# mit-han-lab/litepose

Hardware: AMD Instinct MI355X
Metric: images/sec end-to-end (backbone+deconv+AE-group), LitePose-XS@256 b64 (higher is better)
Workload: dtype f32

## Files before the change

### litepose_amd/csrc/engine.cpp

```cpp
#include <hip/hip_runtime.h>

#include <cmath>
#include <cstdio>
#include <cstdint>
#include <cstring>
#include <map>
#include <string>
#include <vector>

#include "../../include/litepose_amd.h"
#include "kernels.h"
#include "plan.h"

using namespace lp_plan;

namespace {

thread_local std::string g_err;
int fail(int code, const std::string& msg) {
    g_err = msg;
    return code;
}
#define HIP_OK(expr)                                                                   \
    do {                                                                               \
        hipError_t e_ = (expr);                                                        \
        if (e_ != hipSuccess)                                                          \
            return fail(LP_ERR_HIP, std::string(#expr) + ": " + hipGetErrorString(e_)); \
    } while (0)

static_assert(ACT_NONE == lp::ACT_NONE && ACT_RELU == lp::ACT_RELU && ACT_RELU6 == lp::ACT_RELU6, "plan.h restates lp::Act");

const char* storage_name(const Net* n) { return n->storage == LP_STORAGE_F16 ? "f16" : "bf16"; }

}

struct lp_net : lp_plan::Net {
    bool finalized = false;
    float* d_weights = nullptr;
    std::vector<char*> last_buf;
    int lastN = 0, lastH = 0, lastW = 0;
    bool profiling = false;
    std::vector<hipEvent_t> events;
    struct ProfEntry { std::string name, kernel; int64_t bytes, flops; int ev0, ev1; int64_t flops_valu; lp::LaunchNote launch; };
    std::vector<ProfEntry> prof_entries;
    int prof_ev = 0;
    static constexpr int MAX_SIDE = 8;
    hipStream_t side[MAX_SIDE] = {};
    hipEvent_t ev_fork = nullptr, ev_join[MAX_SIDE] = {};
    int nstreams = 0;
    int opt_mb16 = 1;
    int opt_mb16_run = 1;
    int opt_mb16_min = 48;
    int opt_mbt = 1, opt_mbt_s2 = 1;
    int opt_mbconv2 = 1;
    int opt_mbtb = 1, opt_mbtb_s2 = 1;
    int opt_pw3d = 1;
    int opt_mbtd = 1;
    int opt_mbtq = 1;
    int opt_headb = 1;
    int opt_headfuse = 1;
    int opt_dwt = 2;
    int opt_stem = 1;
    int opt_diag_dwpw = 0;
    struct OptEntryT { const char* key; int lo, hi; int lp_net::*field; };
    static const std::vector<OptEntryT>& options();
    std::vector<char> last_stored;
    struct CalibLayer { std::string bn; int C, div; size_t off; };
    struct Calib {
        lp_net* raw = nullptr;
        std::vector<CalibLayer> layers;
        std::map<std::string, int> index;
        std::vector<float> h_bn;
        float* d_bn = nullptr;
        double momentum = 0.1;
        int64_t steps = 0;
        bool uploaded = false;
    };
    Calib* calib = nullptr;
};

namespace {

size_t buf_elems(const lp_net* n, int b, int N, int H, int W, size_t esz) {
    const int d = n->bufs.div[b];
    const size_t f = (size_t)N * n->bufs.ch[b] * (H / d) * (W / d), q = 256 / esz;
    return (f + q - 1) / q * q;
}
size_t buf_floats(const lp_net* n, int b, int N, int H, int W) { return buf_elems(n, b, N, H, W, sizeof(float)); }

size_t buf_bytes(const lp_net* n, int b, int N, int H, int W) {
    const size_t esz = n->storage != LP_STORAGE_F32 ? sizeof(uint16_t) : sizeof(float);
    return buf_elems(n, b, N, H, W, esz) * esz;
}

int size_multiple(const lp_net* n) {
    int m = 16;
    for (int d : n->bufs.div) m = std::max(m, d);
    return m;
}

int check_size(const lp_net* n, int H, int W) {
    const int m = size_multiple(n);
    if (H < m || W < m || (H % m) || (W % m))
        return fail(LP_ERR_INVALID_ARG, "H and W must be positive multiples of " + std::to_string(m) +
                                            " (the deepest plane of this net is 1/" + std::to_string(m) + " of the input)");
    return LP_OK;
}

}

extern "C" {

const char* lp_last_error(void) { return g_err.c_str(); }
void lp_set_error_(const char* msg) { g_err = msg ? msg : ""; }
const char* lp_version(void) { return "litepose_amd 0.1 (gfx950, fp32 planar)"; }

int lp_net_create(lp_net** out, const lp_arch* a) {
    if (!out || !a) return fail(LP_ERR_INVALID_ARG, "null argument");
    lp_net* n = new lp_net();
    if (const int rc = init_arch(*n, *a)) {
        delete n;
        return fail(rc, lp_plan::last_error());
    }
    *out = n;
    return LP_OK;
}

static void calib_release(lp_net* n) {
    if (!n->calib) return;
    if (n->calib->d_bn) (void)hipFree(n->calib->d_bn);
    lp_net_destroy(n->calib->raw);
    delete n->calib;
    n->calib = nullptr;
}

void lp_net_destroy(lp_net* n) {
// ... 183 lines not shown
    const float* Wt;
    bool f32, f16;
    float* f(int b) const { return reinterpret_cast<float*>(buf[b]); }
    const OpBase& op(size_t i) const { return f32 ? static_cast<const OpBase&>(n->ops[i]) : n->bops[i]; }
    Cost cost(size_t i, CostPart part = COST_OP) const {
        return f32 ? op_cost(n->ops[i], 4, false, NB, H, W, part) : op_cost(n->bops[i], 2, n->bops[i].out_f32, NB, H, W);
    }
    int mark(const std::string& name, const Cost& k) const { return prof_mark(n, s, name, k); }
};
struct Planes { int ih, iw, oh, ow; };
Planes planes(const Part& c, const OpBase& o) { return {c.H / o.in_div, c.W / o.in_div, c.H / o.out_div, c.W / o.out_div}; }

struct Rule {
    int (*launch)(const Part&, size_t i);
    std::string (*name)(const OpBase& first, const OpBase& second, const OpBase& last);
    int64_t (*bytes)(const Part&, size_t i);
};

std::string block_name(const OpBase& o, const OpBase& d, const OpBase& last) {
    const std::string nm = o.name + "+" + d.name.substr(d.name.rfind('.', d.name.find('+')) + 1);
    if (&last == &d) return nm;
    const std::string pfx = o.name.substr(0, o.name.rfind('.'));
    const std::string lpf = last.name.substr(0, last.name.rfind('.', last.name.find('+')));
    return pfx + "-" + lpf.substr(lpf.rfind('.') + 1) + nm.substr(pfx.size());
}
std::string blockb_name(const OpBase& o, const OpBase&, const OpBase&) { return o.name + "+dw+point_conv"; }
std::string stem_name(const OpBase&, const OpBase&, const OpBase&) { return "stem.conv3x3s2+dw3+pw"; }
std::string dwpw3_name(const OpBase& dw, const OpBase&, const OpBase&) { return dw.name + "+pw"; }
std::string headb_name(const OpBase&, const OpBase& second, const OpBase& pw) {
    return "final." + pw.name.substr(6, pw.name.find('.', 6) - 6) + (&second == &pw ? ".dw5+pw" : ".dw5+dw5+pw");
}
std::string head_name(const OpBase& dw, const OpBase& second, const OpBase& pw) {
    if (&second != &pw && dw.name.substr(0, dw.name.find('.')) != "final_refined") return pw.name;
    return headb_name(dw, second, pw);
}
std::string half_name(const OpBase& d, CostPart part) {
    if (part == COST_DW_HALF) return d.name.substr(0, d.name.find('+'));
    return d.name.substr(0, d.name.rfind('.', d.name.find('+'))) + ".point_conv";
}


bool is_block(const std::vector<Op>& ops, size_t i) {
    return ops[i].type == OP_PW && ops[i].fuse_next && i + 1 < ops.size() && ops[i + 1].type == OP_DWPW;
}

int rule_mb16(const Part& c, size_t i) {
    const lp_net* n = c.n;
    if (!is_block(n->ops, i)) return 0;
    const Op &o = n->ops[i], &d = n->ops[i + 1];
    const Planes pl = planes(c, o);
    if (!(n->opt_mb16 && c.NB >= n->opt_mb16_min && o.ws_off && d.ws_off && d.wrow_off &&
          lp::mb16_supported(o.Ca, o.Cout, d.Cout, pl.ih, pl.iw, d.K, d.S, d.res >= 0)))
        return 0;
    const float* Wt = c.Wt;
    lp::Mb16Run r;
    memset(&r, 0, sizeof(r));
    for (size_t k = i; k + 1 < n->ops.size() && r.nblocks < lp::MB16_MAX_RUN; k += 2) {
        const Op &e = n->ops[k], &p = n->ops[k + 1];
        if (e.type != OP_PW || !e.fuse_next || p.type != OP_DWPW || !e.ws_off || !p.ws_off || !p.wrow_off) break;
        if (k > i) {
            if (d.res < 0 || p.res != e.inA || e.inA != n->ops[k - 1].out || e.Ca != o.Ca ||
                e.Cout != o.Cout || p.Cout != d.Cout || p.K != d.K || p.S != d.S ||
                e.in_div != o.in_div || p.out_div != d.out_div || !n->opt_mb16_run)
                break;
        } else if (d.res >= 0 && d.res != o.inA) break;
        const int b = r.nblocks++;
        r.w1s[b] = Wt + e.ws_off; r.b1f[b] = Wt + e.b_off; r.wrow[b] = Wt + p.wrow_off;
        r.w2s[b] = Wt + p.ws_off; r.b2f[b] = Wt + p.b2_off; r.out[b] = c.f(p.out);
        if (d.res < 0) break;
    }
    if (r.nblocks < 1 || !lp::launch_mb16(c.f(o.inA), r, d.res >= 0, c.NB, o.Ca, o.Cout, d.Cout, pl.ih, pl.iw, d.K, d.S, c.s))
        return 0;
    return 2 * r.nblocks;
}

int rule_mbt(const Part& c, size_t i) {
    const lp_net* n = c.n;
    if (!is_block(n->ops, i)) return 0;
    const Op &o = n->ops[i], &d = n->ops[i + 1];
    const Planes pl = planes(c, o);
    const float *Wt = c.Wt, *res = d.res >= 0 ? c.f(d.res) : nullptr;
    return ((o.ws_off && d.ws_off && d.wrow_off &&
             lp::launch_mbt(c.f(o.inA), Wt + o.ws_off, Wt + o.b_off, Wt + d.wrow_off, Wt + d.ws_off, Wt + d.b2_off, res,
                            c.f(d.out), c.NB, o.Ca, o.Cout, d.Cout, pl.ih, pl.iw, d.K, d.S, c.s, n->opt_mbt, n->opt_mbt_s2)) ||
            lp::launch_mbconv(c.f(o.inA), Wt + o.w_off, Wt + o.b_off, Wt + d.w_off, Wt + d.b_off, Wt + d.w2_off,
                              Wt + d.b2_off, res, c.f(d.out), c.NB, o.Ca, o.Cout, d.Cout, pl.ih, pl.iw, d.K, d.S, c.s,
                              d.wpair_off ? Wt + d.wpair_off : nullptr, o.ws_off ? Wt + o.ws_off : nullptr,
                              d.wrow_off ? Wt + d.wrow_off : nullptr, n->opt_mbconv2)) ? 2 : 0;
}

int rule_stem3(const Part& c, size_t i) {
    const lp_net* n = c.n;
    const Op& o = n->ops[i];
    if (!(n->opt_stem && o.type == OP_STEM && i + 2 < n->ops.size() && n->ops[i + 1].type == OP_DW &&
          n->ops[i + 2].type == OP_PW && o.st_w0))
        return 0;
    const Op &dw = n->ops[i + 1], &pw = n->ops[i + 2];
    const float* Wt = c.Wt;
    return lp::launch_stem3(c.x, Wt + o.st_w0, Wt + o.b_off, Wt + o.st_w1, Wt + dw.b_off, Wt + o.st_w2, Wt + o.st_b2,
                            c.f(pw.out), c.NB, c.H, c.W, pw.Cout, c.flip_from, c.x_batch, c.s) ? 3 : 0;
}

int rule_dwpw3(const Part& c, size_t i) {
    const lp_net* n = c.n;
    const Op& o = n->ops[i];
    if (!(o.type == OP_DW && o.K == 3 && o.S == 1 && o.act == lp::ACT_RELU6 && i + 1 < n->ops.size())) return 0;
    const Op& pw = n->ops[i + 1];
    if (!(pw.type == OP_PW && pw.inA == o.out && pw.inB < 0 && pw.res < 0 && pw.act == lp::ACT_NONE && pw.has_bias)) return 0;
    const Planes pl = planes(c, o);
    const float* Wt = c.Wt;
    return lp::launch_dwpw(c.f(o.inA), Wt + o.w_off, Wt + o.b_off, Wt + pw.w_off, Wt + pw.b_off, nullptr, c.f(pw.out), c.NB,
                           o.Ca, pl.ih, pl.iw, o.K, o.S, pw.Cout, c.s, n->opt_diag_dwpw) ? 2 : 0;
}

int rule_head(const Part& c, size_t i) {
    const lp_net* n = c.n;
    const std::vector<Op>& ops = n->ops;
    const Op& o = ops[i];
    if (!(n->opt_headfuse && o.type == OP_DW && o.S == 1 && o.act == lp::ACT_RELU && i + 1 < ops.size())) return 0;
    const Op& a = ops[i + 1];
    const Op *d2 = nullptr, *pw = nullptr;
    if (o.K == 5 && a.type == OP_PW && a.inA == o.out && a.inB < 0 && a.res < 0 && a.act == lp::ACT_NONE &&
        (a.out == n->out0_buf || a.out == n->out1_buf))
        pw = &a;
    else if (i + 2 < ops.size() && a.type == OP_DW && ops[i + 2].type == OP_PW && ops[i + 2].inA == o.out &&
             ops[i + 2].inB == a.out && a.S == 1 && o.K == a.K && a.act == lp::ACT_RELU)
        d2 = &a, pw = &ops[i + 2];
    else
        return 0;
    const Planes pl = planes(c, o);
    const float* Wt = c.Wt;
    if (!lp::launch_headfuse(c.f(o.inA), o.Ca, d2 ? c.f(d2->inA) : nullptr, d2 ? d2->Ca : 0,
                             o.wpair_off ? Wt + o.wpair_off : nullptr, d2 && d2->wpair_off ? Wt + d2->wpair_off : nullptr,
                             Wt + pw->w_off, c.f(pw->out), c.NB, pl.oh, pl.ow, o.K, pw->Cout, c.s))
        return 0;
    return d2 ? 3 : 2;
}

const Rule F32_RULES[] = {{rule_mb16, block_name, nullptr}, {rule_mbt, block_name, nullptr}, {rule_stem3, stem_name, nullptr},
                          {rule_dwpw3, dwpw3_name, nullptr}, {rule_head, head_name, nullptr}};

int launch_op_f32(const Part& c, size_t i) {
    const lp_net* n = c.n;
    const Op& o = n->ops[i];
    const Planes pl = planes(c, o);
    const int ih = pl.ih, iw = pl.iw, oh = pl.oh, ow = pl.ow, NB = c.NB;
    const float* Wt = c.Wt;
    hipStream_t s = c.s;
    switch (o.type) {
        case OP_STEM:
            lp::launch_stem(c.x, Wt + o.w_off, Wt + o.b_off, c.f(o.out), NB, c.H, c.W, c.flip_from, c.x_batch, s);
            break;
        case OP_DW:
            lp::launch_dw(c.f(o.inA), Wt + o.w_off, Wt + o.wdup_off, Wt + o.b_off, c.f(o.out), NB, o.Ca, ih, iw, o.K, o.S,
                          o.act, s);
            break;
        case OP_PW:
            lp::launch_pw(c.f(o.inA), o.Ca, o.inB >= 0 ? c.f(o.inB) : nullptr, o.Cb, Wt + o.w_off,
                          o.has_bias ? Wt + o.b_off : nullptr, o.res >= 0 ? c.f(o.res) : nullptr, c.f(o.out), NB, oh * ow,
                          o.Cout, o.act, s, o.ws_off ? Wt + o.ws_off : nullptr, n->opt_pw3d);
            break;
        case OP_DECONV: {
            float* inB = o.inB >= 0 ? c.f(o.inB) : nullptr;
            if (o.w3_off && deconv4_enabled() && o.w4_off &&
                lp::launch_deconv4x3(c.f(o.inA), o.Ca, inB, o.Cb, Wt + o.w4_off, Wt + o.b3_off, c.f(o.out), NB, ih, iw,
                                     o.Cout, s)) {
            } else if (o.w3_off && deconv4_enabled())
// ... 360 lines not shown
    if (steps_out) *steps_out = steps;
    if (steps > 0) return lp_net_finalize(n, 1);
    return LP_OK;
}

static const OpBase* find_tap(const lp_net* n, const char* name) {
    const OpBase* hit = nullptr;
    auto match = [&](const OpBase& o) { if (!hit && (o.tap == name || o.name == name)) hit = &o; };
    for (const Op& o : n->ops) match(o);
    for (const BOp& o : n->bops) if (!o.out_f32) match(o);
    return hit;
}

int64_t lp_net_tap(const lp_net* n, const char* name, float* d_dst, void* stream) {
    if (!n || !name || n->last_buf.empty()) return fail(LP_ERR_INVALID_ARG, "no forward has run");
    const OpBase* o = find_tap(n, name);
    if (!o) return fail(LP_ERR_UNKNOWN_KEY, std::string("unknown tap ") + name);
    const int d = n->bufs.div[o->out];
    const int hw = (n->lastH / d) * (n->lastW / d);
    const int64_t cnt = (int64_t)n->lastN * n->bufs.ch[o->out] * hw;
    if (n->storage != LP_STORAGE_F32) {
        if ((size_t)o->out >= n->last_stored.size() || !n->last_stored[o->out])
            return fail(LP_ERR_UNSUPPORTED, std::string("tap ") + name + ": the last forward did not store this "
                        "tensor (it lives inside a fused block launch; option \"mbtb\" = 0 runs one launch per op)");
        if (d_dst)
            lp::launch_octet_to_planar(n->last_buf[o->out], d_dst, n->lastN, n->bufs.ch[o->out], hw,
                                       (hipStream_t)stream, n->storage == LP_STORAGE_F16);
    } else if (d_dst) {
        hipError_t e = hipMemcpyAsync(d_dst, n->last_buf[o->out], (size_t)cnt * sizeof(float),
                                      hipMemcpyDeviceToDevice, (hipStream_t)stream);
        if (e != hipSuccess) return fail(LP_ERR_HIP, hipGetErrorString(e));
    }
    return cnt;
}

int64_t lp_net_tap_offset(const lp_net* n, const char* name, int NB, int H, int W, int64_t* count) {
    if (!n || !name || !n->finalized) return fail(LP_ERR_INVALID_ARG, "net not finalized");
    if (n->storage != LP_STORAGE_F32) return fail(LP_ERR_UNSUPPORTED, "fp32 storage only");
    if (NB < 1) return fail(LP_ERR_INVALID_ARG, "NB must be positive");
    if (const int rc = check_size(n, H, W)) return rc;
    const OpBase* o = find_tap(n, name);
    if (!o) return fail(LP_ERR_UNKNOWN_KEY, std::string("unknown tap ") + name);
    if (o->out == n->out0_buf || o->out == n->out1_buf) return fail(LP_ERR_UNSUPPORTED, "caller-owned output");
    size_t off = 0;
    for (int b = 0; b < o->out; ++b) off += buf_floats(n, b, NB, H, W);
    const int d = n->bufs.div[o->out];
    if (count) *count = (int64_t)NB * n->bufs.ch[o->out] * (H / d) * (W / d);
    return (int64_t)(off * sizeof(float));
}

int lp_net_set_storage(lp_net* n, int storage) {
    if (!n || (storage != LP_STORAGE_F32 && storage != LP_STORAGE_BF16 && storage != LP_STORAGE_F16))
        return fail(LP_ERR_INVALID_ARG, "storage must be LP_STORAGE_F32, LP_STORAGE_BF16 or LP_STORAGE_F16");
    if (n->calib) return fail(LP_ERR_INVALID_ARG, "a calibration is open on this handle: lp_calib_end() first");
    if (n->arch.family == 1 && storage != LP_STORAGE_F32)
        return fail(LP_ERR_UNSUPPORTED, "lp_net_set_storage: the pose_resnet family (lp_arch.family = 1) runs in fp32 storage "
                                        "only: its dense k x k convolutions have no 16-bit kernels yet");
    if (storage != n->storage) {
        n->storage = storage;
        n->finalized = false;
        n->last_buf.clear();
    }
    return LP_OK;
}

int lp_net_get_storage(const lp_net* n) { return n ? n->storage : LP_ERR_INVALID_ARG; }

int lp_round16(const float* src, float* dst, int64_t count, int storage) {
    if ((!src || !dst) && count > 0) return fail(LP_ERR_INVALID_ARG, "null argument");
    if (storage != LP_STORAGE_BF16 && storage != LP_STORAGE_F16)
        return fail(LP_ERR_INVALID_ARG, "storage must be LP_STORAGE_BF16 or LP_STORAGE_F16");
    for (int64_t i = 0; i < count; ++i) dst[i] = round16(storage, src[i]);
    return LP_OK;
}

typedef lp_net::OptEntryT OptEntry;
const std::vector<OptEntry>& lp_net::options() {
    static const std::vector<OptEntry> t = {
        {"mb16", 0, 1, &lp_net::opt_mb16},
        {"mb16_run", 0, 1, &lp_net::opt_mb16_run},
        {"mb16_min", 0, 65536, &lp_net::opt_mb16_min},
        {"mbt", 0, 3, &lp_net::opt_mbt},
        {"mbt_s2", 0, 1, &lp_net::opt_mbt_s2},
        {"mbconv2", 0, 1, &lp_net::opt_mbconv2},
        {"mbtb", 0, 1, &lp_net::opt_mbtb},
        {"mbtb_s2", 0, 1, &lp_net::opt_mbtb_s2},
        {"mbtq", 0, 2, &lp_net::opt_mbtq},
        {"mbtd", 0, 1, &lp_net::opt_mbtd},
        {"pw3d", 0, 2, &lp_net::opt_pw3d},
        {"headb", 0, 1, &lp_net::opt_headb},
        {"headfuse", 0, 1, &lp_net::opt_headfuse},
        {"dwt", 0, 2, &lp_net::opt_dwt},
        {"stem", 0, 1, &lp_net::opt_stem},
        {"diag_dwpw", 0, 2, &lp_net::opt_diag_dwpw},
    };
    return t;
}

int lp_net_set_option(lp_net* n, const char* key, int value) {
    if (!n || !key) return fail(LP_ERR_INVALID_ARG, "null argument");
    for (const OptEntry& e : lp_net::options())
        if (!strcmp(key, e.key)) {
            if (value < e.lo || value > e.hi) return fail(LP_ERR_INVALID_ARG, std::string("option ") + key + ": value out of range");
#ifndef LP_DIAG_BUILD
            if (e.field == &lp_net::opt_diag_dwpw && value != 0)
                return fail(LP_ERR_UNSUPPORTED, "option diag_dwpw: the self-checking dwpw_kernel exists only in the diagnostics "
                                                "flavour of the library (python -m litepose_amd.build --flavour diag, "
                                                "LP_NATIVE_FLAVOUR=diag)");
#endif
            n->*(e.field) = value;
            return LP_OK;
        }
    return fail(LP_ERR_UNKNOWN_KEY, std::string("unknown option ") + key);
}

int lp_net_get_option(const lp_net* n, const char* key) {
    if (!n || !key) return fail(LP_ERR_INVALID_ARG, "null argument");
    for (const OptEntry& e : lp_net::options())
        if (!strcmp(key, e.key)) return n->*(e.field);
    return fail(LP_ERR_UNKNOWN_KEY, std::string("unknown option ") + key);
}

int lp_diag_read(uint32_t* words, int cap_words, int clear) {
    const int n = lp::dwpw_diag_read(words, cap_words, clear != 0);
    if (n == -2) return fail(LP_ERR_UNSUPPORTED, "lp_diag_read: no diagnostic kernel in this library (build --flavour diag)");
    if (n < 0) return fail(LP_ERR_HIP, "lp_diag_read: copy from the device log failed");
    return n;
}

int lp_phase_trace_read(uint64_t* words, int nwg) {
    static_assert(sizeof(unsigned long long) == sizeof(uint64_t), "");
    const int n = lp::phase_trace_read(reinterpret_cast<unsigned long long*>(words), nwg);
    if (n == -2) return fail(LP_ERR_UNSUPPORTED, "lp_phase_trace_read: no phase trace in this library (build --flavour trace)");
    if (n < 0) return fail(LP_ERR_HIP, "lp_phase_trace_read: bad count / copy from the device table failed");
    return n;
}

int lp_wg_trace_read(uint64_t* words, int nwg, int select_cexp) {
    if (nwg < 0 || nwg > 16384) return fail(LP_ERR_INVALID_ARG, "lp_wg_trace_read: 0..16384 workgroups");
    const int n = lp::wg_trace_read(reinterpret_cast<unsigned long long*>(words), nwg, select_cexp);
    if (n == -2) return fail(LP_ERR_UNSUPPORTED, "lp_wg_trace_read: no trace in this library (build --flavour trace)");
    if (n < 0) return fail(LP_ERR_HIP, "lp_wg_trace_read: copy failed");
    return n;
}

int lp_net_set_streams(lp_net* n, int k) {
    if (!n || k < 1 || k > lp_net::MAX_SIDE) return fail(LP_ERR_INVALID_ARG, "streams must be 1..8");
    n->nstreams = k;
    return LP_OK;
}

int lp_net_set_profiling(lp_net* n, int enable) {
    if (!n) return fail(LP_ERR_INVALID_ARG, "null net");
    n->profiling = enable != 0;
    return LP_OK;
}

int lp_net_profile(const lp_net* n, char names[][48], float* ms, int64_t* alg_bytes, int64_t* flops,
                   int cap) {
    return lp_net_profile2(n, names, ms, alg_bytes, flops, nullptr, cap);
}

int lp_net_profile2(const lp_net* n, char names[][48], float* ms, int64_t* alg_bytes, int64_t* flops,
                    int64_t* flops_valu, int cap) {
    if (!n || !n->profiling || n->prof_entries.empty())
        return fail(LP_ERR_INVALID_ARG, "profiling not enabled / no forward yet");
// ... 24 lines not shown
```

### litepose_amd/csrc/kernels.h

```cpp
#pragma once
#include <hip/hip_runtime.h>
#include <stdint.h>

namespace lp {

enum Act { ACT_NONE = 0, ACT_RELU = 1, ACT_RELU6 = 2 };

bool uses_scratch(const void* kernel_fn);

extern thread_local const char* last_kernel_tag;

struct LaunchNote { int grid = 0, block = 0, lds = 0, wgs_per_cu = 0; };
extern thread_local LaunchNote last_launch;
extern thread_local bool launch_notes;
void note_launch(const void* fn, dim3 grid, dim3 block, size_t lds);
#define LP_LAUNCH(kern, grid, block, lds, stream, ...)                                                   \
    do {                                                                                                 \
        if (lp::launch_notes) lp::note_launch(reinterpret_cast<const void*>(kern), grid, block, lds);    \
        hipLaunchKernelGGL(kern, grid, block, lds, stream, __VA_ARGS__);                                 \
    } while (0)

#ifndef LP_NO_LDS_DMA
#define LP_STAGE_LOAD(reg, src, dst)                                                                  \
    __builtin_amdgcn_global_load_lds((const __attribute__((address_space(1))) void*)(src),           \
                                     (__attribute__((address_space(3))) void*)(dst), 16, 0, 0)
#define LP_STAGE_STORE(reg, dst, lane) ((void)0)
#define LP_STAGE_DRAIN() asm volatile("s_waitcnt vmcnt(0)" ::: "memory")
#else
#define LP_STAGE_LOAD(reg, src, dst) ((reg) = *(src))
#define LP_STAGE_STORE(reg, dst, lane) ((dst)[lane] = (reg))
#define LP_STAGE_DRAIN() ((void)0)
#endif

#ifdef LP_CLAIM_CU
#define LP_OWN_CU() asm volatile("; own the CU: whole register budget, no co-resident waves" ::: "v255")
#else
#define LP_OWN_CU() ((void)0)
#endif

void launch_stem(const float* x, const float* w, const float* b, float* out,
                 int N, int H, int W, int flip_from, int x_batch, hipStream_t s);

bool launch_stem3(const float* x, const float* w0t, const float* b0, const float* w1t, const float* b1,
                  const float* w2t, const float* b2, float* out, int N, int H, int W, int c0, int flip_from,
                  int x_batch, hipStream_t s);

bool launch_stem3b(const float* x, const float* w0t, const float* b0, const float* w1t, const float* b1,
                   const float* w2t, const float* b2, void* out, int N, int H, int W, int c0, int flip_from,
                   int x_batch, hipStream_t s, bool f16 = false);

void launch_dw(const float* in, const float* w, const float* wdup, const float* b, float* out,
               int N, int C, int H, int W, int K, int S, int act, hipStream_t s);

void launch_pw(const float* inA, int Ca, const float* inB, int Cb,
               const float* wp, const float* b, const float* res, float* out,
               int N, int HW, int Cout, int act, hipStream_t s, const void* wsplit = nullptr, int pw3d_mode = 1);
struct PwTile { int NB, PXV; };
PwTile pw_tile_choice(int N, int Ca, int Cb, int Cout, int HW, bool has_res);

bool launch_dwpw(const float* in, const float* wdw, const float* bdw, const float* wp, const float* bias,
                 const float* res, float* out, int N, int C, int H, int W, int K, int S, int Cout,
                 hipStream_t s, int diag = 0);
int dwpw_diag_read(unsigned* host, int cap_words, bool clear);

bool launch_headfuse(const float* inA, int Ca, const float* inB, int Cb, const float* wpairA, const float* wpairB,
                     const float* wp, float* out, int N, int H, int W, int K, int Cout, hipStream_t s);

bool launch_mbconv(const float* x, const float* w1p, const float* b1f, const float* wdw,
                   const float* bdw, const float* w2p, const float* b2f, const float* res, float* out,
                   int N, int Cin, int Cexp, int Cout, int H, int W, int K, int S, hipStream_t s,
                   const float* wdw_pair = nullptr, const void* w1_split = nullptr, const void* wdw_rows = nullptr,
                   int mbconv2 = 1);

constexpr int MB16_MAX_RUN = 10;
struct Mb16Run {
    const void* w1s[MB16_MAX_RUN];
    const float* b1f[MB16_MAX_RUN];
    const void* wrow[MB16_MAX_RUN];
    const void* w2s[MB16_MAX_RUN];
    const float* b2f[MB16_MAX_RUN];
    float* out[MB16_MAX_RUN];
    int nblocks;
};
bool mb16_supported(int Cin, int Cexp, int Cout, int H, int W, int K, int S, bool res);
bool launch_mb16(const float* x, const Mb16Run& run, bool res, int N, int Cin, int Cexp, int Cout, int H, int W,
                 int K, int S, hipStream_t s);

bool launch_mbt(const float* x, const void* w1s, const float* b1f, const void* wrow, const void* w2s,
                const float* b2f, const float* res, float* out, int N, int Cin, int Cexp, int Cout, int H, int W,
                int K, int S, hipStream_t s, int mode = 1, int mode_s2 = 1);

void launch_deconv_pair(const float* inA, int Ca, const float* inB, int Cb,
                        const float* w, const float* b, float* out,
                        int N, int h, int w_, int Cout, hipStream_t s);

void launch_deconv4(const float* inA, int Ca, const float* inB, int Cb, const float* wq, const float* bias,
                    float* out, int N, int h, int w_, int Cout, hipStream_t s);
bool launch_deconv4x3(const float* inA, int Ca, const float* inB, int Cb, const void* ws, const float* bias,
                      float* out, int N, int h, int w_, int Cout, hipStream_t s);
void launch_deconv_mfma(const float* inA, int Ca, const float* inB, int Cb, const float* wp,
                        const float* bias, float* out, int N, int h, int w_, int Cout, hipStream_t s);

bool launch_convk3(const float* inA, int Ca, const float* inB, int Cb, const void* ws, const float* bias, float* out,
                   int N, int IH, int IW, int K, int S, int ups, int Cout, int act, int flip_from, int x_batch,
                   hipStream_t s);

void launch_stem_raw(const float* x, const float* w, float* out, int N, int H, int W, hipStream_t s);
void launch_deconv_raw(const float* inA, int Ca, const float* inB, int Cb, const float* w, float* out, int N, int h,
                       int w_, int Cout, hipStream_t s);
struct BnCut { int S, chunk, vec; };
BnCut bn_cut(int N, int C, int HW);
size_t bn_partial_doubles(int N, int C, int HW);
void launch_bn_stats(const float* x, double* part, int N, int C, int HW, hipStream_t s);
void launch_bn_apply(float* x, const float* res, const double* part, float* bn, int N, int C, int HW, int act,
                     double momentum, double eps, hipStream_t s);

void launch_stemb(const float* x, const float* w, const float* b, void* out, int N, int H, int W, int flip_from,
                  int x_batch, hipStream_t s, bool f16 = false);
bool launch_dwt(const void* in, const void* wt, const float* wb, void* out, int N, int C, int H, int W, int K, int act,
                hipStream_t s, bool f16 = false);
bool launch_dwb(const void* in, const float* w, void* out, int N, int C, int H, int W, int K, int S, int act,
                hipStream_t s, bool f16 = false);
bool launch_pwb(const void* inA, int Ca, const void* inB, int Cb, const void* wf, const float* bias, const void* res,
                void* out, int N, int HW, int Cout, int act, bool out_f32, hipStream_t s, bool f16 = false);
bool launch_headb(const void* inA, int Ca, const void* inB, int Cb, const void* wtA, const float* wbA, const void* wtB,
                  const float* wbB, const void* wf, float* out, int N, int H, int W, int K, int Cout, hipStream_t s,
                  bool f16 = false);
bool launch_mbtb(const void* x, const void* w1, const float* b1f, const void* wrow, const void* w2, const float* b2f,
                 const void* res, void* out, int N, int Cin, int Cexp, int Cout, int H, int W, int K, int S,
                 hipStream_t s, int mode = 1, int mode_s2 = 1, int mode_q = 1, const void* wrow2 = nullptr, int mode_d = 1,
                 bool f16 = false);
int phase_trace_read(unsigned long long* host, int nwg);
int wg_trace_read(unsigned long long* host, int nwg, int sel);
bool launch_deconvb(const void* inA, int Ca, const void* inB, int Cb, const void* wf, const float* bias, void* out,
                    int N, int h, int w_, int Cout, hipStream_t s, bool f16 = false);
void launch_octet_to_planar(const void* in, float* out, int N, int C, int HW, hipStream_t s, bool f16 = false);

struct ParseParams {
    int J, M;
    double det_thr, tag_thr;
    int use_det_val, ignore_too_much, nms_k, tag_per_joint;
    int joint_order[32];
};

struct FlipIndex { int v[32]; };
bool launch_tta_stage(const float* out0, const float* out1, const float* out0f, const float* out1f,
                      int N, int J, int C0, int C1, int tag_off, int h0, int w0, int h1, int w1,
                      const FlipIndex& flip_index, float* mid, hipStream_t s, const float* add0 = nullptr,
                      const float* add1 = nullptr, const float* add0f = nullptr, const float* add1f = nullptr);
void launch_maps_accumulate(float* acc, const float* src, long count, hipStream_t s);
bool launch_tta_project(const float* mid, int N, int J, int h1, int w1, int Hp, int Wp, int T,
                        float* det, float* tag, hipStream_t s);
constexpr int MAX_SCALES = 8;
struct ScaleMid {
    const float* mid;
    int h1, w1;
};
static_assert(sizeof(ScaleMid) == 16, "ScaleMid must match lp_scale_mid (16 bytes)");
struct ScaleTable { ScaleMid s[MAX_SCALES]; };
void launch_tta_merge_scales(const ScaleTable& t, int S, int first_unit, int N, int J, int T, int project2image,
                             int Hf, int Wf, float* det, float* tag, hipStream_t s);

bool launch_peaks_topk(const float* det, const float* tag, int N, int J, int H, int W, int T,
                       const ParseParams& p, float* val_k, int* ind_k, float* tag_k, hipStream_t s,
                       const float* mid = nullptr);
void launch_group(const float* val_k, const int* ind_k, const float* tag_k, int N, int W, int T,
                  const ParseParams& p, int pcap, float* ans, int* count, hipStream_t s);
void launch_adjust_scores(const float* det, const float* tag, int N, int J, int H, int W, int T,
                          int pcap, int do_adjust, float* ans, const int* count, float* scores,
                          float* prev, unsigned* miss, hipStream_t s);
void launch_refine(const float* det, const float* tag, int N, int J, int H, int W, int T, int pcap,
                   float* ans, const int* count, const float* prev, const unsigned* miss,
                   hipStream_t s);
// ... 117 lines not shown
```

### litepose_amd/csrc/mbtile_kernels.hip

```cpp
#include "kernels.h"
#include "dw7.h"
#include "split3.h"

#include <cstdlib>

namespace lp {

constexpr int MT_RS = 26;
constexpr int MT_PAIR = 22 * MT_RS * 2 + 4;
constexpr int MT_E_FLOATS = 16 * MT_PAIR;
constexpr int MT_CELLS = 22 * 22;

template <int CK, int NMT> struct MTW {
    static constexpr int N1 = CK * 3 * 64, N2 = NMT * 2 * 3 * 64, N3 = 64, N4 = 16 * 28;
    static constexpr int NTOT = N1 + N2 + N3 + N4;
    static constexpr int NLD = (NTOT + 511) / 512;
    static constexpr size_t LDS_BYTES = (size_t)MT_E_FLOATS * 4 + (size_t)(NTOT + N4) * 16;
};

__device__ __forceinline__ int mt_xcd_contiguous_id(int id, int n) {
    const int q = n >> 3, r = n & 7;
    const int xcd = id & 7, slot = id >> 3;
    return xcd * q + min(xcd, r) + slot;
}
// ... 128 lines not shown
        {
            const f32x4* bp = reinterpret_cast<const f32x4*>(W2 + WG::N2) + half * 4;
            f32x4 bq[4];
#pragma unroll
            for (int q = 0; q < 4; ++q) bq[q] = bp[q];
#pragma unroll
            for (int gi = 0; gi < 2; ++gi) {
                if (ein[gi]) {
#pragma unroll
                    for (int q = 0; q < 4; ++q)
#pragma unroll
                        for (int e = 0; e < 4; e += 2) {
                            const int cc = 4 * half + e + 8 * q;
                            const float v0 = fminf(fmaxf(d[gi][4 * q + e] + bq[q][e], 0.f), 6.f);
                            const float v1 = fminf(fmaxf(d[gi][4 * q + e + 1] + bq[q][e + 1], 0.f), 6.f);
                            const f32x2 pv = {xok[gi] ? v0 : 0.f, xok[gi] ? v1 : 0.f};
                            *reinterpret_cast<f32x2*>(E + (cc >> 1) * MT_PAIR + ecell[gi]) = pv;
                        }
                }
            }
        }
        __syncthreads();
        stage_load(ch);
        {
            const int kp = wave * 2 + dwpair;
            const f32x4* wl = reinterpret_cast<const f32x4*>(WD + (ch & 1) * WG::N4) + kp * 28;
            float* ep = E + kp * MT_PAIR;
            f32x2 a0[4] = {{0.f, 0.f}, {0.f, 0.f}, {0.f, 0.f}, {0.f, 0.f}};
            f32x2 a1[4] = {{0.f, 0.f}, {0.f, 0.f}, {0.f, 0.f}, {0.f, 0.f}};
            dw7_s1_2x4<MT_RS * 2>(ep + dwoff, wl, a0, a1);
            const f32x4 wbias = wl[3];
            const float b0 = wbias[2], b1 = wbias[3];
            f32x4 o00, o01, o10, o11;
            o00[0] = fminf(fmaxf(a0[0][0] + b0, 0.f), 6.f); o00[1] = fminf(fmaxf(a0[0][1] + b1, 0.f), 6.f);
            o00[2] = fminf(fmaxf(a0[1][0] + b0, 0.f), 6.f); o00[3] = fminf(fmaxf(a0[1][1] + b1, 0.f), 6.f);
            o01[0] = fminf(fmaxf(a0[2][0] + b0, 0.f), 6.f); o01[1] = fminf(fmaxf(a0[2][1] + b1, 0.f), 6.f);
            o01[2] = fminf(fmaxf(a0[3][0] + b0, 0.f), 6.f); o01[3] = fminf(fmaxf(a0[3][1] + b1, 0.f), 6.f);
            o10[0] = fminf(fmaxf(a1[0][0] + b0, 0.f), 6.f); o10[1] = fminf(fmaxf(a1[0][1] + b1, 0.f), 6.f);
            o10[2] = fminf(fmaxf(a1[1][0] + b0, 0.f), 6.f); o10[3] = fminf(fmaxf(a1[1][1] + b1, 0.f), 6.f);
            o11[0] = fminf(fmaxf(a1[2][0] + b0, 0.f), 6.f); o11[1] = fminf(fmaxf(a1[2][1] + b1, 0.f), 6.f);
            o11[2] = fminf(fmaxf(a1[3][0] + b0, 0.f), 6.f); o11[3] = fminf(fmaxf(a1[3][1] + b1, 0.f), 6.f);
            *reinterpret_cast<f32x4*>(ep + dwout) = o00;
            *reinterpret_cast<f32x4*>(ep + dwout + 4) = o01;
            *reinterpret_cast<f32x4*>(ep + dwout + MT_RS * 2) = o10;
            *reinterpret_cast<f32x4*>(ep + dwout + MT_RS * 2 + 4) = o11;
        }
        stage_store(ch);
        __syncthreads();
#pragma unroll
        for (int ks2 = 0; ks2 < 2; ++ks2) {
            u32x4 fh, fm, fl;
#pragma unroll
            for (int j = 0; j < 4; ++j) {
                const f32x2 v = *reinterpret_cast<const f32x2*>(E + (8 * ks2 + 4 * half + j) * MT_PAIR + pcell);
                const Split3 p3 = split3_pair(v[0], v[1]);
                fh[j] = p3.h; fm[j] = p3.m; fl[j] = p3.l;
            }
#pragma unroll
            for (int mt = 0; mt < NMT; ++mt) {
                const u32x4* wl = W2 + (mt * 2 + ks2) * 3 * 64 + lane;
                u32x4 a[3];
#pragma unroll
                for (int t = 0; t < 3; ++t) a[t] = wl[t * 64];
                acc[mt] = mma6(a, fh, fm, fl, acc[mt]);
            }
        }
    }
    const int oy = y0 + prow, ox = x0 + pcol;
    if (oy < H && ox < W) {
        const long o = (long)oy * W + ox;
        float* ob = out + (long)n * Cout * HW + o;
        const float* rb = x + (long)n * Cin * HW + o;
#pragma unroll
        for (int mt = 0; mt < NMT; ++mt) {
            const f32x4* bp = reinterpret_cast<const f32x4*>(b2f + (mt * 2 + half) * 16);
#pragma unroll
            for (int q = 0; q < 4; ++q) {
                if (mt * 32 + 8 * q >= Cout) break;
                const f32x4 bq = bp[q];
#pragma unroll
                for (int e = 0; e < 4; ++e) {
                    const int co = mt * 32 + 4 * half + e + 8 * q;
                    float v = acc[mt][4 * q + e] + bq[e];
                    if (RES) v += rb[(long)co * HW];
                    ob[(long)co * HW] = v;
                }
            }
        }
    }
}

constexpr int S2_RS = 44;
constexpr int S2_ODD = 22;
constexpr int S2_ROWS = 21, S2_COLS = 37;
constexpr int S2_PAIR = S2_ROWS * S2_RS * 2;
constexpr int S2_E_FLOATS = 16 * S2_PAIR;
constexpr int S2_CELLS = S2_ROWS * S2_COLS;
constexpr int S2_NG = (S2_CELLS + 31) / 32;
constexpr int S2_GPW = (S2_NG + 7) / 8;

template <int CK, int NMT> struct S2W {
    static constexpr int N1 = CK * 3 * 64, N2 = NMT * 2 * 3 * 64, N3 = 64, N4 = 16 * 28;
    static constexpr int NTOT = N1 + N2 + N3 + N4;
    static constexpr int NLD = (NTOT + 511) / 512;
    static constexpr size_t LDS_BYTES = (size_t)S2_E_FLOATS * 4 + (size_t)(NTOT + N4) * 16;
};

template <int CK, int NMT>
__global__ __launch_bounds__(512, 2) void mbt_s2_kernel(
    const float* __restrict__ x,
    const u32x4* __restrict__ w1s,
    const float* __restrict__ b1f,
    const f32x4* __restrict__ wrow,
    const u32x4* __restrict__ w2s,
    const float* __restrict__ b2f,
    float* __restrict__ out,
    int Cexp, int Cout, int H, int W, int OH, int OW, int tilesX, int tilesY, int xcd_remap) {
    extern __shared__ __attribute__((aligned(16))) float E[];
    LP_OWN_CU();
    constexpr int Cin = CK * 16;
    const int lane = threadIdx.x & 63;
    const int wave = __builtin_amdgcn_readfirstlane(threadIdx.x >> 6);
    const int half = lane >> 5, pl = lane & 31;
    const int unit = xcd_remap ? mt_xcd_contiguous_id(blockIdx.x, gridDim.x) : (int)blockIdx.x;
    const int tq = unit / tilesX;
    const int tx = unit - tq * tilesX;
    const int n = tq / tilesY;
    const int ty = tq - n * tilesY;
    const int ox0 = tx * 16, oy0 = ty * 8;
    const int x0 = 2 * ox0 - 3, y0 = 2 * oy0 - 3;
    const long HW = (long)H * W;
    const int nchunks = Cexp >> 5, KS2 = Cexp >> 4;
    using WG = S2W<CK, NMT>;
    u32x4* W1 = reinterpret_cast<u32x4*>(E + S2_E_FLOATS);
    u32x4* W2 = W1 + WG::N1;
    u32x4* WD = W2 + WG::N2 + WG::N3;

    u32x4 stg[WG::NLD];
    auto stage_addr = [&](int c, int j, const u32x4*& src, u32x4*& dst) -> bool {
        const int e0 = 64 * wave + 512 * j;
        if (e0 >= WG::NTOT) return false;
        const int ca = max(c, 0), cb = min(c + 1, nchunks - 1), dpar = (c + 1) & 1;
                dst = W1 + e0;
        if (e0 < WG::N1) src = w1s + (long)cb * WG::N1 + e0 + lane;
        else if (e0 < WG::N1 + WG::N2) {
            const int f0 = e0 - WG::N1, seg = f0 / 192, within = f0 - seg * 192;
            src = w2s + ((long)(seg >> 1) * KS2 + 2 * ca + (seg & 1)) * 192 + within + lane;
        } else if (e0 < WG::N1 + WG::N2 + WG::N3) {
            src = reinterpret_cast<const u32x4*>(b1f) + (long)cb * 8 + min(lane, 7);
        } else {
            src = reinterpret_cast<const u32x4*>(wrow) + (long)cb * WG::N4 + (e0 - WG::N1 - WG::N2 - WG::N3) + lane;
            dst += dpar * WG::N4;
        }
        return true;
    };
    auto stage_load = [&](int c) {
#pragma unroll
        for (int j = 0; j < WG::NLD; ++j) {
            const u32x4* src;
            u32x4* dst;
            if (stage_addr(c, j, src, dst)) LP_STAGE_LOAD(stg[j], src, dst);
        }
    };
    auto stage_store = [&](int c) {
#pragma unroll
        for (int j = 0; j < WG::NLD; ++j) {
// ... 128 lines not shown
            for (int mt = 0; mt < NMT; ++mt) {
                const u32x4* wl = W2 + (mt * 2 + pks) * 3 * 64 + lane;
                u32x4 a[3];
#pragma unroll
                for (int t = 0; t < 3; ++t) a[t] = wl[t * 64];
                acc[mt] = mma6(a, fh, fm, fl, acc[mt]);
            }
        }
    }
    __syncthreads();
    if (pks == 1) {
#pragma unroll
        for (int mt = 0; mt < NMT; ++mt)
#pragma unroll
            for (int r = 0; r < 16; ++r) E[((pt * NMT + mt) * 16 + r) * 64 + lane] = acc[mt][r];
    }
    __syncthreads();
    if (pks == 0) {
        const int orow = ppx >> 4, ocol = ppx & 15;
        const int oy = oy0 + orow, ox = ox0 + ocol;
        const long OHW = (long)OH * OW;
        if (oy < OH && ox < OW) {
            float* ob = out + (long)n * Cout * OHW + (long)oy * OW + ox;
#pragma unroll
            for (int mt = 0; mt < NMT; ++mt) {
                const f32x4* bp = reinterpret_cast<const f32x4*>(b2f + (mt * 2 + half) * 16);
#pragma unroll
                for (int q = 0; q < 4; ++q) {
                    if (mt * 32 + 8 * q >= Cout) break;
                    const f32x4 bq = bp[q];
#pragma unroll
                    for (int e = 0; e < 4; ++e) {
                        const int co = mt * 32 + 4 * half + e + 8 * q;
                        const float v = (acc[mt][4 * q + e] + E[((pt * NMT + mt) * 16 + 4 * q + e) * 64 + lane]) + bq[e];
                        ob[(long)co * OHW] = v;
                    }
                }
            }
        }
    }
}

template <int CK, int NMT>
static void launch_mbt_s2_t(const float* x, const void* w1s, const float* b1f, const void* wrow, const void* w2s,
                            const float* b2f, float* out, int N, int Cexp, int Cout, int H, int W, int xcd,
                            hipStream_t s) {
    const size_t lds = S2W<CK, NMT>::LDS_BYTES;
    static bool attr = false;
    if (!attr) {
        (void)hipFuncSetAttribute(reinterpret_cast<const void*>(mbt_s2_kernel<CK, NMT>),
                                  hipFuncAttributeMaxDynamicSharedMemorySize, (int)lds);
        attr = true;
    }
    const int OH = H / 2, OW = W / 2;
    const int tilesX = (OW + 15) / 16, tilesY = (OH + 7) / 8;
    LP_LAUNCH((mbt_s2_kernel<CK, NMT>), dim3(N * tilesX * tilesY), dim3(512), lds, s, x, (const u32x4*)w1s,
                       b1f, (const f32x4*)wrow, (const u32x4*)w2s, b2f, out, Cexp, Cout, H, W, OH, OW, tilesX, tilesY,
                       xcd);
}

template <int CK, int NMT>
static void launch_mbt_t(const float* x, const void* w1s, const float* b1f, const void* wrow, const void* w2s,
                         const float* b2f, bool res, float* out, int N, int Cexp, int Cout, int H, int W,
                         int xcd, hipStream_t s) {
    const size_t lds = MTW<CK, NMT>::LDS_BYTES;
    static bool attr = false;
    if (!attr) {
        (void)hipFuncSetAttribute(reinterpret_cast<const void*>(mbt_kernel<CK, NMT, true>),
                                  hipFuncAttributeMaxDynamicSharedMemorySize, (int)lds);
        (void)hipFuncSetAttribute(reinterpret_cast<const void*>(mbt_kernel<CK, NMT, false>),
                                  hipFuncAttributeMaxDynamicSharedMemorySize, (int)lds);
        attr = true;
    }
    const int tilesX = (W + 15) / 16, tilesY = (H + 15) / 16;
    const dim3 grid(N * tilesX * tilesY);
    if (res)
        LP_LAUNCH((mbt_kernel<CK, NMT, true>), grid, dim3(512), lds, s, x, (const u32x4*)w1s, b1f,
                           (const f32x4*)wrow, (const u32x4*)w2s, b2f, out, Cexp, Cout, H, W, tilesX, tilesY, xcd);
    else
        LP_LAUNCH((mbt_kernel<CK, NMT, false>), grid, dim3(512), lds, s, x, (const u32x4*)w1s, b1f,
                           (const f32x4*)wrow, (const u32x4*)w2s, b2f, out, Cexp, Cout, H, W, tilesX, tilesY, xcd);
}

bool launch_mbt(const float* x, const void* w1s, const float* b1f, const void* wrow, const void* w2s,
                const float* b2f, const float* res, float* out, int N, int Cin, int Cexp, int Cout, int H, int W,
                int K, int S, hipStream_t s, int mode, int mode_s2) {
    if (mode == 0) return false;
    constexpr int xcd = 1;
    if (K == 7 && S == 2 && !res && w1s && b1f && wrow && w2s && b2f) {
        if (!mode_s2) return false;
        if ((Cin & 15) || Cin > 32 || (Cexp & 31) || (Cout & 7) || Cout > 64 || (H & 1) || (W & 1)) return false;
        if (H < 16 || W < 16) return false;
        const int ck2 = Cin >> 4, nmt2 = (Cout + 31) >> 5;
        last_kernel_tag = "mbt_s2_kernel";
#define LP_GO2(CKV, NMTV)                                                                                   \
        if (ck2 == CKV && nmt2 == NMTV) {                                                                   \
            if (uses_scratch((const void*)mbt_s2_kernel<CKV, NMTV>)) return false;                          \
            launch_mbt_s2_t<CKV, NMTV>(x, w1s, b1f, wrow, w2s, b2f, out, N, Cexp, Cout, H, W, xcd, s);      \
            return true;                                                                                    \
        }
        LP_GO2(1, 1) LP_GO2(1, 2) LP_GO2(2, 1) LP_GO2(2, 2)
#undef LP_GO2
        return false;
    }
    if (K != 7 || S != 1 || !w1s || !b1f || !wrow || !w2s || !b2f) return false;
    if ((Cin & 15) || Cin > 48 || (Cexp & 31) || (Cout & 7) || Cout > 64) return false;
    if (res && (res != x || Cin != Cout)) return false;
    if (H < 17 && W < 17) return false;
    if (mode == 3) return false;
    if (mode == 1 && Cin < 32) return false;
    if ((long)N * ((W + 15) / 16) * ((H + 15) / 16) > 0x7fffffffL) return false;
    const int ck = Cin >> 4, nmt = (Cout + 31) >> 5;
    last_kernel_tag = "mbt_kernel";
#define LP_GO(CKV, NMTV)                                                                                   \
    if (ck == CKV && nmt == NMTV) {                                                                        \
        if (uses_scratch(res ? (const void*)mbt_kernel<CKV, NMTV, true> : (const void*)mbt_kernel<CKV, NMTV, false>)) \
            return false;                                                                                  \
        launch_mbt_t<CKV, NMTV>(x, w1s, b1f, wrow, w2s, b2f, res != nullptr, out, N, Cexp, Cout, H, W,     \
                                xcd, s);                                                                   \
        return true;                                                                                       \
    }
    LP_GO(1, 1) LP_GO(2, 1) LP_GO(2, 2) LP_GO(3, 1) LP_GO(3, 2)
#undef LP_GO
    return false;
}

}
```

Measured before the change: 22900.

## Add full-width 16x32 strip variant of fused MBConv tile kernel for W=32

Adds a strip form of the fused expand/depthwise-7x7/project MBConv kernel that covers a full 32-wide row strip of 16 rows per workgroup instead of 16x16 tiles. It is selected when W is 32 and the strip grid still fills the device's CUs. The goal is to cut halo recomputation and redundant weight staging across horizontally adjacent tiles, at the cost of a larger LDS footprint and each wave computing two output rows, which raises register pressure.

```diff
diff --git a/litepose_amd/csrc/engine.cpp b/litepose_amd/csrc/engine.cpp
--- a/litepose_amd/csrc/engine.cpp
+++ b/litepose_amd/csrc/engine.cpp
@@ -52,6 +52,7 @@
     int opt_mb16_run = 1;
     int opt_mb16_min = 48;
     int opt_mbt = 1, opt_mbt_s2 = 1;
+    int opt_mbt_strip = 1;
     int opt_mbconv2 = 1;
     int opt_mbtb = 1, opt_mbtb_s2 = 1;
     int opt_pw3d = 1;
@@ -401,7 +402,8 @@
     const float *Wt = c.Wt, *res = d.res >= 0 ? c.f(d.res) : nullptr;
     return ((o.ws_off && d.ws_off && d.wrow_off &&
              lp::launch_mbt(c.f(o.inA), Wt + o.ws_off, Wt + o.b_off, Wt + d.wrow_off, Wt + d.ws_off, Wt + d.b2_off, res,
-                            c.f(d.out), c.NB, o.Ca, o.Cout, d.Cout, pl.ih, pl.iw, d.K, d.S, c.s, n->opt_mbt, n->opt_mbt_s2)) ||
+                            c.f(d.out), c.NB, o.Ca, o.Cout, d.Cout, pl.ih, pl.iw, d.K, d.S, c.s, n->opt_mbt, n->opt_mbt_s2,
+                            n->opt_mbt_strip)) ||
             lp::launch_mbconv(c.f(o.inA), Wt + o.w_off, Wt + o.b_off, Wt + d.w_off, Wt + d.b_off, Wt + d.w2_off,
                               Wt + d.b2_off, res, c.f(d.out), c.NB, o.Ca, o.Cout, d.Cout, pl.ih, pl.iw, d.K, d.S, c.s,
                               d.wpair_off ? Wt + d.wpair_off : nullptr, o.ws_off ? Wt + o.ws_off : nullptr,
@@ -928,6 +930,7 @@
         {"mb16_min", 0, 65536, &lp_net::opt_mb16_min},
         {"mbt", 0, 3, &lp_net::opt_mbt},
         {"mbt_s2", 0, 1, &lp_net::opt_mbt_s2},
+        {"mbt_strip", 0, 2, &lp_net::opt_mbt_strip},
         {"mbconv2", 0, 1, &lp_net::opt_mbconv2},
         {"mbtb", 0, 1, &lp_net::opt_mbtb},
         {"mbtb_s2", 0, 1, &lp_net::opt_mbtb_s2},
diff --git a/litepose_amd/csrc/kernels.h b/litepose_amd/csrc/kernels.h
--- a/litepose_amd/csrc/kernels.h
+++ b/litepose_amd/csrc/kernels.h
@@ -88,7 +88,7 @@
 
 bool launch_mbt(const float* x, const void* w1s, const float* b1f, const void* wrow, const void* w2s,
                 const float* b2f, const float* res, float* out, int N, int Cin, int Cexp, int Cout, int H, int W,
-                int K, int S, hipStream_t s, int mode = 1, int mode_s2 = 1);
+                int K, int S, hipStream_t s, int mode = 1, int mode_s2 = 1, int mode_strip = 1);
 
 void launch_deconv_pair(const float* inA, int Ca, const float* inB, int Cb,
                         const float* w, const float* b, float* out,
diff --git a/litepose_amd/csrc/mbtile_kernels.hip b/litepose_amd/csrc/mbtile_kernels.hip
--- a/litepose_amd/csrc/mbtile_kernels.hip
+++ b/litepose_amd/csrc/mbtile_kernels.hip
@@ -234,6 +234,243 @@
                 for (int e = 0; e < 4; ++e) {
                     const int co = mt * 32 + 4 * half + e + 8 * q;
                     float v = acc[mt][4 * q + e] + bq[e];
+                    if (RES) v += rb[(long)co * HW];
+                    ob[(long)co * HW] = v;
+                }
+            }
+        }
+    }
+}
+
+constexpr int MS_RS = 42;
+constexpr int MS_PAIR = 22 * MS_RS * 2 + 4;
+constexpr int MS_E_FLOATS = 16 * MS_PAIR;
+
+template <int CK, int NMT> struct MSW : MTW<CK, NMT> {
+    static constexpr size_t LDS_BYTES = (size_t)MS_E_FLOATS * 4 + (size_t)(MTW<CK, NMT>::NTOT + MTW<CK, NMT>::N4) * 16;
+};
+
+template <int CK, int NMT, bool RES, int ROWS>
+__global__ __launch_bounds__(512, 2) void mbt_kernel(
+    const float* __restrict__ x,
+    const u32x4* __restrict__ w1s, const float* __restrict__ b1f, const f32x4* __restrict__ wrow,
+    const u32x4* __restrict__ w2s, const float* __restrict__ b2f,
+    float* __restrict__ out,
+    int Cexp, int Cout, int H, int stripsY, int xcd_remap) {
+    static_assert(ROWS == 16, "a strip is 16 output rows");
+    extern __shared__ __attribute__((aligned(16))) float E[];
+    LP_OWN_CU();
+    constexpr int Cin = CK * 16, W = 32;
+    const int lane = threadIdx.x & 63;
+    const int wave = __builtin_amdgcn_readfirstlane(threadIdx.x >> 6);
+    const int half = lane >> 5, pl = lane & 31;
+    const int unit = xcd_remap ? mt_xcd_contiguous_id(blockIdx.x, gridDim.x) : (int)blockIdx.x;
+    const int n = unit / stripsY;
+    const int y0 = (unit - n * stripsY) * 16;
+    const long HW = (long)H * W;
+    const int nchunks = Cexp >> 5, KS2 = Cexp >> 4;
+    using WG = MSW<CK, NMT>;
+    u32x4* W1 = reinterpret_cast<u32x4*>(E + MS_E_FLOATS);
+    u32x4* W2 = W1 + WG::N1;
+    u32x4* WD = W2 + WG::N2 + WG::N3;
+
+    u32x4 stg[WG::NLD];
+    auto stage_addr = [&](int c, int j, const u32x4*& src, u32x4*& dst) -> bool {
+        const int e0 = 64 * wave + 512 * j;
+        if (e0 >= WG::NTOT) return false;
+        const int ca = max(c, 0), cb = min(c + 1, nchunks - 1), dpar = (c + 1) & 1;
+        dst = W1 + e0;
+        if (e0 < WG::N1) src = w1s + (long)cb * WG::N1 + e0 + lane;
+        else if (e0 < WG::N1 + WG::N2) {
+            const int f0 = e0 - WG::N1, seg = f0 / 192, within = f0 - seg * 192;
+            src = w2s + ((long)(seg >> 1) * KS2 + 2 * ca + (seg & 1)) * 192 + within + lane;
+        } else if (e0 < WG::N1 + WG::N2 + WG::N3) {
+            src = reinterpret_cast<const u32x4*>(b1f) + (long)cb * 8 + min(lane, 7);
+        } else {
+            src = reinterpret_cast<const u32x4*>(wrow) + (long)cb * WG::N4 + (e0 - WG::N1 - WG::N2 - WG::N3) + lane;
+            dst += dpar * WG::N4;
+        }
+        return true;
+    };
+    auto stage_load = [&](int c) {
+#pragma unroll
+        for (int j = 0; j < WG::NLD; ++j) {
+            const u32x4* src;
+            u32x4* dst;
+            if (stage_addr(c, j, src, dst)) LP_STAGE_LOAD(stg[j], src, dst);
+        }
+    };
+    auto stage_store = [&](int c) {
+#pragma unroll
+        for (int j = 0; j < WG::NLD; ++j) {
+            const u32x4* src;
+            u32x4* dst;
+            if (stage_addr(c, j, src, dst)) LP_STAGE_STORE(stg[j], dst, lane);
+        }
+        LP_STAGE_DRAIN();
+    };
+    stage_load(-1);
+
+    {
+        const f32x4 z = {0.f, 0.f, 0.f, 0.f};
+        for (int i = threadIdx.x; i < MS_E_FLOATS / 4; i += 512) reinterpret_cast<f32x4*>(E)[i] = z;
+    }
+
+    u32x4 xh[3][CK], xm[3][CK], xl[3][CK];
+    int trow[3];
+    bool gok[3];
+    trow[0] = 2 * wave + 3;
+    trow[1] = 2 * wave + 4;
+    trow[2] = wave < 3 ? wave : wave == 7 ? 19 : wave == 4 ? 20 : wave == 5 ? 21 : -1;
+#pragma unroll
+    for (int gi = 0; gi < 3; ++gi) {
+        const int yy = y0 - 3 + trow[gi];
+        gok[gi] = trow[gi] >= 0 && yy >= 0 && yy < H;
+#pragma unroll
+        for (int ks = 0; ks < CK; ++ks) xh[gi][ks] = xm[gi][ks] = xl[gi][ks] = u32x4{0u, 0u, 0u, 0u};
+        if (gok[gi]) {
+            const float* sp = x + ((long)n * Cin + 8 * half) * HW + (long)yy * W + pl;
+#pragma unroll
+            for (int ks = 0; ks < CK; ++ks) {
+                float v[8];
+#pragma unroll
+                for (int c = 0; c < 8; ++c) v[c] = sp[(long)(ks * 16 + c) * HW];
+#pragma unroll
+                for (int j = 0; j < 4; ++j) {
+                    const Split3 p3 = split3_pair(v[2 * j], v[2 * j + 1]);
+                    xh[gi][ks][j] = p3.h; xm[gi][ks][j] = p3.m; xl[gi][ks][j] = p3.l;
+                }
+            }
+        }
+    }
+    f32x16 acc[NMT][2];
+#pragma unroll
+    for (int mt = 0; mt < NMT; ++mt)
+#pragma unroll
+        for (int g = 0; g < 2; ++g)
+#pragma unroll
+            for (int r = 0; r < 16; ++r) acc[mt][g][r] = 0.f;
+
+    const int dq = pl >> 2;
+    const int dwpair = (0x66 >> dq) & 1;
+    const int dwrp = ((0x96 >> dq) & 1) + 2 * half;
+    const int strip = (lane & 3) + 4 * ((dq >> 1) & 1);
+    const int dwoff = (2 * dwrp * MS_RS + strip * 4) * 2;
+    const int dwout = ((2 * dwrp + 3) * MS_RS + 4 + strip * 4) * 2;
+    constexpr int PASS = 8 * MS_RS * 2;
+    const int pcell = ((2 * wave + 3) * MS_RS + pl + 4) * 2;
+
+    stage_store(-1);
+    __syncthreads();
+    for (int ch = 0; ch < nchunks; ++ch) {
+        {
+            u32x4 a[CK][3];
+#pragma unroll
+            for (int ks = 0; ks < CK; ++ks)
+#pragma unroll
+                for (int t = 0; t < 3; ++t) a[ks][t] = W1[(ks * 3 + t) * 64 + lane];
+            const f32x4* bp = reinterpret_cast<const f32x4*>(W2 + WG::N2) + half * 4;
+            f32x4 bq[4];
+#pragma unroll
+            for (int q = 0; q < 4; ++q) bq[q] = bp[q];
+#pragma unroll
+            for (int gi = 0; gi < 3; ++gi) {
+                if (!gok[gi]) continue;
+                f32x16 d;
+#pragma unroll
+                for (int r = 0; r < 16; ++r) d[r] = 0.f;
+#pragma unroll
+                for (int ks = 0; ks < CK; ++ks) d = mma6(a[ks], xh[gi][ks], xm[gi][ks], xl[gi][ks], d);
+                float* ec = E + (trow[gi] * MS_RS + pl + 4) * 2;
+#pragma unroll
+                for (int q = 0; q < 4; ++q)
+#pragma unroll
+                    for (int e = 0; e < 4; e += 2) {
+                        const int cc = 4 * half + e + 8 * q;
+                        const float v0 = fminf(fmaxf(d[4 * q + e] + bq[q][e], 0.f), 6.f);
+                        const float v1 = fminf(fmaxf(d[4 * q + e + 1] + bq[q][e + 1], 0.f), 6.f);
+                        *reinterpret_cast<f32x2*>(ec + (cc >> 1) * MS_PAIR) = f32x2{v0, v1};
+                    }
+            }
+        }
+        __syncthreads();
+        stage_load(ch);
+        {
+            const int kp = wave * 2 + dwpair;
+            const f32x4* wl = reinterpret_cast<const f32x4*>(WD + (ch & 1) * WG::N4) + kp * 28;
+            float* ep = E + kp * MS_PAIR;
+            const f32x4 wbias = wl[3];
+            const float b0 = wbias[2], b1 = wbias[3];
+            f32x4 o[2][4];
+#pragma unroll
+            for (int p = 0; p < 2; ++p) {
+                f32x2 a0[4] = {{0.f, 0.f}, {0.f, 0.f}, {0.f, 0.f}, {0.f, 0.f}};
+                f32x2 a1[4] = {{0.f, 0.f}, {0.f, 0.f}, {0.f, 0.f}, {0.f, 0.f}};
+                dw7_s1_2x4<MS_RS * 2>(ep + dwoff + p * PASS, wl, a0, a1);
+#pragma unroll
+                for (int i = 0; i < 4; ++i) {
+                    o[p][i >> 1][2 * (i & 1)] = fminf(fmaxf(a0[i][0] + b0, 0.f), 6.f);
+                    o[p][i >> 1][2 * (i & 1) + 1] = fminf(fmaxf(a0[i][1] + b1, 0.f), 6.f);
+                    o[p][2 + (i >> 1)][2 * (i & 1)] = fminf(fmaxf(a1[i][0] + b0, 0.f), 6.f);
+                    o[p][2 + (i >> 1)][2 * (i & 1) + 1] = fminf(fmaxf(a1[i][1] + b1, 0.f), 6.f);
+                }
+#pragma unroll
+                for (int k = 0; k < 4; ++k) asm volatile("" : "+v"(o[p][k]) : : "memory");
+            }
+            const f32x4 z = {0.f, 0.f, 0.f, 0.f};
+#pragma unroll
+            for (int p = 0; p < 2; ++p) {
+                const int oy = y0 + 2 * (dwrp + 4 * p);
+                float* op = ep + dwout + p * PASS;
+                *reinterpret_cast<f32x4*>(op) = oy < H ? o[p][0] : z;
+                *reinterpret_cast<f32x4*>(op + 4) = oy < H ? o[p][1] : z;
+                *reinterpret_cast<f32x4*>(op + MS_RS * 2) = oy + 1 < H ? o[p][2] : z;
+                *reinterpret_cast<f32x4*>(op + MS_RS * 2 + 4) = oy + 1 < H ? o[p][3] : z;
+            }
+        }
+        stage_store(ch);
+        __syncthreads();
+#pragma unroll
+        for (int ks2 = 0; ks2 < 2; ++ks2) {
+            u32x4 fh[2], fm[2], fl[2];
+#pragma unroll
+            for (int g = 0; g < 2; ++g)
+#pragma unroll
+                for (int j = 0; j < 4; ++j) {
+                    const f32x2 v = *reinterpret_cast<const f32x2*>(E + (8 * ks2 + 4 * half + j) * MS_PAIR + pcell +
+                                                                    g * MS_RS * 2);
+                    const Split3 p3 = split3_pair(v[0], v[1]);
+                    fh[g][j] = p3.h; fm[g][j] = p3.m; fl[g][j] = p3.l;
+                }
+#pragma unroll
+            for (int mt = 0; mt < NMT; ++mt) {
+                const u32x4* wl = W2 + (mt * 2 + ks2) * 3 * 64 + lane;
+                u32x4 a[3];
+#pragma unroll
+                for (int t = 0; t < 3; ++t) a[t] = wl[t * 64];
+#pragma unroll
+                for (int g = 0; g < 2; ++g) acc[mt][g] = mma6(a, fh[g], fm[g], fl[g], acc[mt][g]);
+            }
+        }
+    }
+#pragma unroll
+    for (int g = 0; g < 2; ++g) {
+        const int oy = y0 + 2 * wave + g;
+        if (oy >= H) continue;
+        const long o = (long)oy * W + pl;
+        float* ob = out + (long)n * Cout * HW + o;
+        const float* rb = x + (long)n * Cin * HW + o;
+#pragma unroll
+        for (int mt = 0; mt < NMT; ++mt) {
+            const f32x4* bp = reinterpret_cast<const f32x4*>(b2f + (mt * 2 + half) * 16);
+#pragma unroll
+            for (int q = 0; q < 4; ++q) {
+                if (mt * 32 + 8 * q >= Cout) break;
+                const f32x4 bq = bp[q];
+#pragma unroll
+                for (int e = 0; e < 4; ++e) {
+                    const int co = mt * 32 + 4 * half + e + 8 * q;
+                    float v = acc[mt][g][4 * q + e] + bq[e];
                     if (RES) v += rb[(long)co * HW];
                     ob[(long)co * HW] = v;
                 }
@@ -528,9 +765,44 @@
                            (const f32x4*)wrow, (const u32x4*)w2s, b2f, out, Cexp, Cout, H, W, tilesX, tilesY, xcd);
 }
 
+template <int CK, int NMT>
+static void launch_mbt_strip_t(const float* x, const void* w1s, const float* b1f, const void* wrow, const void* w2s,
+                               const float* b2f, bool res, float* out, int N, int Cexp, int Cout, int H, int xcd,
+                               hipStream_t s) {
+    const size_t lds = MSW<CK, NMT>::LDS_BYTES;
+    static_assert(MSW<CK, NMT>::LDS_BYTES <= 160 * 1024, "the strip form's E tile and weight stage must fit the CU's LDS");
+    static bool attr = false;
+    if (!attr) {
+        (void)hipFuncSetAttribute(reinterpret_cast<const void*>(mbt_kernel<CK, NMT, true, 16>),
+                                  hipFuncAttributeMaxDynamicSharedMemorySize, (int)lds);
+        (void)hipFuncSetAttribute(reinterpret_cast<const void*>(mbt_kernel<CK, NMT, false, 16>),
+                                  hipFuncAttributeMaxDynamicSharedMemorySize, (int)lds);
+        attr = true;
+    }
+    const int stripsY = (H + 15) / 16;
+    const dim3 grid(N * stripsY);
+    if (res)
+        LP_LAUNCH((mbt_kernel<CK, NMT, true, 16>), grid, dim3(512), lds, s, x, (const u32x4*)w1s, b1f,
+                           (const f32x4*)wrow, (const u32x4*)w2s, b2f, out, Cexp, Cout, H, stripsY, xcd);
+    else
+        LP_LAUNCH((mbt_kernel<CK, NMT, false, 16>), grid, dim3(512), lds, s, x, (const u32x4*)w1s, b1f,
+                           (const f32x4*)wrow, (const u32x4*)w2s, b2f, out, Cexp, Cout, H, stripsY, xcd);
+}
+
+static int device_cu_count() {
+    static const int cus = [] {
+        int dev = 0, v = 0;
+        if (hipGetDevice(&dev) != hipSuccess ||
+            hipDeviceGetAttribute(&v, hipDeviceAttributeMultiprocessorCount, dev) != hipSuccess || v <= 0)
+            return 1 << 30;
+        return v;
+    }();
+    return cus;
+}
+
 bool launch_mbt(const float* x, const void* w1s, const float* b1f, const void* wrow, const void* w2s,
                 const float* b2f, const float* res, float* out, int N, int Cin, int Cexp, int Cout, int H, int W,
-                int K, int S, hipStream_t s, int mode, int mode_s2) {
+                int K, int S, hipStream_t s, int mode, int mode_s2, int mode_strip) {
     if (mode == 0) return false;
     constexpr int xcd = 1;
     if (K == 7 && S == 2 && !res && w1s && b1f && wrow && w2s && b2f) {
@@ -566,6 +838,17 @@
                                 xcd, s);                                                                   \
         return true;                                                                                       \
     }
+    if (W == 32 && mode_strip && (mode_strip == 2 || (long)N * ((H + 15) / 16) >= device_cu_count())) {
+#define LP_GOS(CKV, NMTV)                                                                                  \
+        if (ck == CKV && nmt == NMTV &&                                                                    \
+            !uses_scratch(res ? (const void*)mbt_kernel<CKV, NMTV, true, 16>                               \
+                              : (const void*)mbt_kernel<CKV, NMTV, false, 16>)) {                          \
+            launch_mbt_strip_t<CKV, NMTV>(x, w1s, b1f, wrow, w2s, b2f, res != nullptr, out, N, Cexp, Cout, H, xcd, s); \
+            return true;                                                                                   \
+        }
+        LP_GOS(1, 1) LP_GOS(2, 1)
+#undef LP_GOS
+    }
     LP_GO(1, 1) LP_GO(2, 1) LP_GO(2, 2) LP_GO(3, 1) LP_GO(3, 2)
 #undef LP_GO
     return false;
```

Result: faster. 23530, median of 6 (+2.8%).
